# lubaroli/sigsvgd

Measured on AMD Instinct MI355X. Metric: SVGD iters/sec, sig-kernel N=1024 T=64 d=7, higher is better.
Workload: dtype f64 static kernel + f32 sweeps and contraction (mixed), f32 I/O

## Files before the change

### sigsvgd_amd/csrc/gram_fast.hip

```cpp
#include <cstdlib>

#include "gram_fast_kernel.h"

namespace sigsvgd {

bool fast_supported(int T, int d, int n) { return n == 0 && T >= 3 && T <= 64 && d <= 16; }

namespace {
inline int grad_nw(int T, int d) { return (d <= 8) ? 8 : 4; }
inline int grad_wg_per_cu(int T, int d) { return (d <= 8 && T <= 32) ? 3 : 1; }
GradGeom fast_geometry(int A, int B, int T, int d, bool sym, int off, int stride, bool fold)
{
    return grad_geometry(A, B, T * d, sym, off, stride, fold, grad_nw(T, d), (long long)device_cu_count() * grad_wg_per_cu(T, d));
}
}

int sym_tile_rows_fast(int T, int d) { return grad_nw(T, d); }

static bool fixed_windows(int T, int want_grad)
{
    if (T != 64 || !want_grad) return false;
    const char *e = getenv("SIGSVGD_SWEEP_WINDOWS");
    return !(e && e[0] == 't');
}

static bool wave_balance(int T, int d, int want_grad, bool sym)
{
    if (!sym || d > 8 || !fast_has_balance<8, true>() || !fixed_windows(T, want_grad)) return false;
    const char *e = getenv("SIGSVGD_WAVE_BALANCE");
    return !(e && e[0] == 'o' && e[1] == 'f');
}

WsPlan fast_plan(int A, int B, int T, int d, int want_grad, bool sym, int off, int stride, bool fold, int kind)
{
    WsPlan w;
    const bool rbf = kind == SIGSVGD_STATIC_RBF;
    w.fixed_windows = rbf && fixed_windows(T, want_grad) ? 1 : 0;
    w.wave_balance = rbf && wave_balance(T, d, want_grad, sym) ? 1 : 0;
    if (d <= 4) w.kflag = w.take(flag_area_bytes(A, B));
    if (want_grad) {
        w.g = fast_geometry(A, B, T, d, sym, off, stride, fold);
        w.rseg = w.take(w.g.rseg_bytes);
        w.cslab = w.take(w.g.cslab_bytes);
    }
    return w;
}

namespace {
int run(const GramProblem &p, const WsPlan &w, bool sym, const TileMap &own, void *out, int out64)
{
    unsigned char *base = nullptr;
    int rc = ws_base(p, w, "fast", base);
    if (rc) return rc;
    FastArgs a{};
    fill_sweep_args(a, p, w, base);
    a.tm = own;
    int tile_rows = 0;
    rc = p.kind == SIGSVGD_STATIC_RBF ? dispatch_variant<0>(p, a, w, out != nullptr, sym, tile_rows)
                                      : fast_radial_dispatch(p, a, w, out != nullptr, sym, tile_rows);
    if (rc) return rc;
    return finish_launch(p, w, base, sym, a.tm, tile_rows, out, out64);
}
}

int fast_launch(const GramProblem &p)
{
    const bool sym = (p.flags & SIGSVGD_FLAG_Y_IS_X) && p.A == p.B;
    const WsPlan w = fast_plan(p.A, p.B, p.T, p.d, p.gradX_out != nullptr, sym, 0, 1, false, p.kind);
    return run(p, w, sym, make_tilemap(1, 0, 1, false), p.gradX_out, p.dtype == SIGSVGD_F64);
}

int fast_sym_partial(const GramProblem &p, int tile_offset, int tile_stride, bool fold, double *grad_partial)
{
    const WsPlan w = fast_plan(p.A, p.B, p.T, p.d, 1, true, tile_offset, tile_stride, fold, p.kind);
    return run(p, w, true, make_tilemap((p.A + grad_nw(p.T, p.d) - 1) / grad_nw(p.T, p.d), tile_offset, tile_stride, fold),
               grad_partial, 1);
}

}

SIG_EXEC_DEBUG_GETTER(fast)
```

### sigsvgd_amd/csrc/gram_fast_kernel.h

```cpp
#pragma once

#include <type_traits>

#include "sig_common.h"

namespace sigsvgd {

#define SIG_PRIO(n)                                                          \
    if (!GRAD || !SYM || (RING == 32 && NW == 4)) __builtin_amdgcn_s_setprio(n);

template <int BAL>
__device__ __forceinline__ void bal_top(bool first)
{
    if constexpr (BAL != 0) {
        if (first) __builtin_amdgcn_s_setprio(1);
    }
}
template <int BAL, int AT>
__device__ __forceinline__ void bal_switch(bool first)
{
    if constexpr (BAL != 0 && (BAL & 3) == AT) {
        if (first) __builtin_amdgcn_s_setprio(0);
        else __builtin_amdgcn_s_setprio(1);
    }
// ... 271 lines not shown
template <int PFIX, int SIGMA0, int NS>
__device__ __forceinline__ void sweep_rev_fixed(float &cur, float &dnA, float &dnB, float &V, const float *g, float *ksl, const float r3)
{
    static_assert((NS == 8 || NS == 5) && SIGMA0 % 8 == 0 && SIGMA0 + NS <= 2 * PFIX - 1, "statement shape");
    float t, y;
    SIG_EXEC_MUST_BE_FULL("sweep_rev_fixed");
    if constexpr (NS == 8)
        asm volatile(SIG_REV_STEP_X("dnA", "dnB", "g7", "k7", SIG_WIN_FIX("7")) SIG_REV_STEP_X("dnB", "dnA", "g6", "k6", SIG_WIN_FIX("6"))
                     SIG_REV_STEP_X("dnA", "dnB", "g5", "k5", SIG_WIN_FIX("5")) SIG_REV_STEP_X("dnB", "dnA", "g4", "k4", SIG_WIN_FIX("4"))
                     SIG_REV_STEP_X("dnA", "dnB", "g3", "k3", SIG_WIN_FIX("3")) SIG_REV_STEP_X("dnB", "dnA", "g2", "k2", SIG_WIN_FIX("2"))
                     SIG_REV_STEP_X("dnA", "dnB", "g1", "k1", SIG_WIN_FIX("1")) SIG_REV_STEP_X("dnB", "dnA", "g0", "k0", SIG_WIN_FIX("0"))
                     "s_mov_b64 exec, -1\n\t"
                     : [cur] "+v"(cur), [dnA] "+v"(dnA), [dnB] "+v"(dnB), [V] "+v"(V), [t] "=&v"(t), [y] "=&v"(y),
                       [k0] "+v"(ksl[0]), [k1] "+v"(ksl[1]), [k2] "+v"(ksl[2]), [k3] "+v"(ksl[3]), [k4] "+v"(ksl[4]),
                       [k5] "+v"(ksl[5]), [k6] "+v"(ksl[6]), [k7] "+v"(ksl[7])
                     : [g0] "v"(g[0]), [g1] "v"(g[1]), [g2] "v"(g[2]), [g3] "v"(g[3]), [g4] "v"(g[4]), [g5] "v"(g[5]),
                       [g6] "v"(g[6]), [g7] "v"(g[7]), [r3] "s"(r3), SIG_WIN_OPS(0), SIG_WIN_OPS(1), SIG_WIN_OPS(2),
                       SIG_WIN_OPS(3), SIG_WIN_OPS(4), SIG_WIN_OPS(5), SIG_WIN_OPS(6), SIG_WIN_OPS(7));
    else
        asm volatile(SIG_REV_STEP_X("dnB", "dnA", "g4", "k4", SIG_WIN_FIX("4"))
                     SIG_REV_STEP_X("dnA", "dnB", "g3", "k3", SIG_WIN_FIX("3")) SIG_REV_STEP_X("dnB", "dnA", "g2", "k2", SIG_WIN_FIX("2"))
                     SIG_REV_STEP_X("dnA", "dnB", "g1", "k1", SIG_WIN_FIX("1")) SIG_REV_STEP_X("dnB", "dnA", "g0", "k0", SIG_WIN_FIX("0"))
                     "s_mov_b64 exec, -1\n\t"
                     : [cur] "+v"(cur), [dnA] "+v"(dnA), [dnB] "+v"(dnB), [V] "+v"(V), [t] "=&v"(t), [y] "=&v"(y),
                       [k0] "+v"(ksl[0]), [k1] "+v"(ksl[1]), [k2] "+v"(ksl[2]), [k3] "+v"(ksl[3]), [k4] "+v"(ksl[4])
                     : [g0] "v"(g[0]), [g1] "v"(g[1]), [g2] "v"(g[2]), [g3] "v"(g[3]), [g4] "v"(g[4]), [r3] "s"(r3),
                       SIG_WIN_OPS(0), SIG_WIN_OPS(1), SIG_WIN_OPS(2), SIG_WIN_OPS(3), SIG_WIN_OPS(4));
}
template <int PFIX, int S0, int S1>
__device__ __forceinline__ void sweep_fwd_fixed_round(float &cur, float &upA, float &upB, float &V, const float *Dsl, float *Ksl, const float r3)
{
    if constexpr (S0 < S1) {
        sweep_fwd_fixed<PFIX, S0, (S1 - S0 < 8 ? S1 - S0 : 8)>(cur, upA, upB, V, Dsl + (S0 & 63), Ksl + (S0 & 63), r3);
        sweep_fwd_fixed_round<PFIX, S0 + 8, S1>(cur, upA, upB, V, Dsl, Ksl, r3);
    }
}
template <int PFIX, int S0, int S1>
__device__ __forceinline__ void sweep_rev_fixed_round(float &cur, float &dnA, float &dnB, float &V, const float *Dsl, float *Ksl, const float r3)
{
    if constexpr (S0 < S1) {
        sweep_rev_fixed_round<PFIX, S0 + 8, S1>(cur, dnA, dnB, V, Dsl, Ksl, r3);
        sweep_rev_fixed<PFIX, S0, (S1 - S0 < 8 ? S1 - S0 : 8)>(cur, dnA, dnB, V, Dsl + (S0 & 63), Ksl + (S0 & 63), r3);
    }
}

template <int RING>
__device__ __forceinline__ double resweep_fwd_fp64(const float (&Dsl)[RING], int P, int lrow)
{
    double cur = 1.0, upprev = 1.0;
    asm volatile("" : "+v"(lrow), "+s"(P));
    const bool rowv = lrow < P;
#pragma unroll
    for (int s0 = 0; s0 < 2 * RING - 3; s0 += 8) {
        if (s0 <= 2 * P - 2) {
#pragma unroll
            for (int s = s0; s < s0 + 8 && s < 2 * RING - 3; ++s) {
                const double up = dpp_shr1_one(cur);
                float gf = Dsl[s & (RING - 1)];
                asm volatile("" : "+v"(gf));
                const double g = (double)gf;
                const double t = cur + up;
                const double nw = (t - upprev) + g * __builtin_fma(g, t + upprev, 1.7320508075688772 * t);
                cur = (rowv && (unsigned)(s - lrow) < (unsigned)P) ? nw : cur;
                upprev = up;
            }
        }
    }
    return cur;
}

__device__ __forceinline__ double rsqrt_ge1(double x)
{
    const double y = __builtin_amdgcn_rsq(x);
    const double e = __builtin_fma(-(x * y), y, 1.0);
    return __builtin_fma(y * e, __builtin_fma(e, 0.375, 0.5), y);
}

constexpr int GS_STRIDE = 65;
constexpr int GS_WAVE = 64 * GS_STRIDE;
using f32x2 = __attribute__((ext_vector_type(2))) float;

__device__ __forceinline__ int gs_index(int slot, int lane) { return slot * GS_STRIDE + lane; }

template <int DPAD, int NW, bool GRAD, bool SYM, bool LP, int RING = 64, int PFIX = 0, int BAL = 0, int RADIAL = 0>
__global__ __launch_bounds__(NW * 64) __attribute__((amdgpu_waves_per_eu(
    GRAD ? ((RING == 32 && NW == 4 && DPAD <= 8) ? 3 : 1) : ((DPAD <= 8) ? 3 : 2),
    GRAD ? ((RING == 32 && NW == 4 && DPAD <= 8) ? 3 : 2) : ((DPAD <= 8) ? 3 : 2)))) void gram_fast_kernel(FastArgsOf<RADIAL> a)
{
    constexpr int DC = LP ? DPAD - 1 : DPAD;
    constexpr int NT = NW * 64;
    constexpr int RM = RING - 1;
    constexpr int RPW = (RING == 32) ? 2 : 1;
    constexpr int NWR = NW * RPW;
    static_assert(RADIAL == 0 || (PFIX == 0 && BAL == 0), "the radial kinds: general windows, no wave balance");
    static_assert(BAL == 0 || (GRAD && SYM && RING == 64 && NW == 8 && PFIX != 0 && (BAL & 3) != 0 && BAL < 8),
                  "wave balance: the symmetric gradient kernels with fixed windows on 8-wave workgroups (the ones SIG_PRIO leaves alone)");
    constexpr int YDS = DPAD + 2;
    constexpr int YFS = (DPAD == 4) ? 12 : DPAD + 4;
    constexpr int GSW = RING * GS_STRIDE;
    __shared__ float Gs_all[GRAD ? NW * GSW : 1];
    __shared__ __align__(16) double yd[2 * RING * YDS];
    __shared__ double ynd[2 * RING];
    __shared__ double yref[DPAD];
    __shared__ __align__(16) float yf[GRAD ? 2 * RING * YFS : 1];

    const int tid = threadIdx.x, lane = tid & 63;
    const int wave = __builtin_amdgcn_readfirstlane(tid >> 6);
    const int lrow = lane & RM;
    const bool bal_first = (BAL & 4) ? wave < NW / 2 : wave >= NW / 2;
    const int T = a.T, d = a.d, P = T - 1, io64 = a.io64;
#ifdef SIGSVGD_PHASE_STAMPS
    unsigned long long ph_[SIG_FAST_PHASES] = {0, 0, 0, 0, 0, 0, 0, 0, 0}, tlast_ = __builtin_amdgcn_s_memtime();
#endif
    int j0 = 0, j1 = 0;
    float *Gs = Gs_all + (GRAD ? wave * GSW : 0);
    const double inv_h = a.inv_h;
    const float m2h = (float)(-2.0 * inv_h * 3.46410161513775459);

    float Ksl[RING];
    double gacc[DPAD];
    double xraw[DPAD];

    constexpr int EPT = (64 * DPAD + NT - 1) / NT;
    constexpr bool RAW_STAGE = GRAD && SYM && RING == 64 && DPAD == 8;
    struct RawElem { unsigned lo, hi; };
    RawElem raw_v[EPT], raw_r[EPT];
    double stage_v[EPT], stage_r[EPT];
    auto load_raw = [&](const void *b, size_t idx) -> RawElem {
        const char *p = static_cast<const char *>(b) + (idx << (io64 ? 3 : 2));
        RawElem r;
        r.lo = *reinterpret_cast<const unsigned *>(p);
        r.hi = 0u;
        if (io64) r.hi = *reinterpret_cast<const unsigned *>(p + 4);
        return r;
    };
    auto raw_value = [&](const RawElem &r) -> double {
        return io64 ? __hiloint2double((int)r.hi, (int)r.lo) : (double)__uint_as_float(r.lo);
    };
    auto stage_load = [&](int j) {
#pragma unroll
        for (int k = 0; k < EPT; ++k) {
            const int e = tid + k * NT;
            const int t = e / DPAD, c = e % DPAD;
            const bool ok = e < RING * DPAD && t < T && c < d && j < a.B;
            if constexpr (RAW_STAGE) {
                raw_v[k] = raw_r[k] = RawElem{0u, 0u};
                if (ok) {
                    raw_v[k] = load_raw(a.Y, ((size_t)j * T + t) * d + c);
                    raw_r[k] = load_raw(a.Y, (size_t)j * T * d + c);
                }
            } else {
                stage_v[k] = ok ? load_any(a.Y, ((size_t)j * T + t) * d + c, io64) : 0.0;
                stage_r[k] = ok ? load_any(a.Y, (size_t)j * T * d + c, io64) : 0.0;
            }
        }
    };
    const double nscale = RADIAL ? inv_h : -inv_h * 1.4426950408889634074;
    auto stage_store = [&]() {
#pragma unroll
        for (int k = 0; k < EPT; ++k) {
            const int e = tid + k * NT;
            if (e < RING * DPAD) {
                const int t = e / DPAD, c = e % DPAD;
                if constexpr (RAW_STAGE) {
                    stage_v[k] = raw_value(raw_v[k]);
                    stage_r[k] = raw_value(raw_r[k]);
                }
                const double v = stage_v[k] - stage_r[k];
                if (!(LP && c == DPAD - 1)) {
                    yd[t * YDS + c] = v;
                    yd[(t + RING) * YDS + c] = v;
                }
                if (GRAD) {
                    yf[t * YFS + c] = (float)v;
                    yf[(t + RING) * YFS + c] = (float)v;
                }
                if (t == 0) yref[c] = stage_r[k];
                double s = v * v * nscale;
#pragma unroll
                for (int off = 1; off < DPAD; off <<= 1) s += __shfl_xor(s, off, 64);
                if (c == 0) {
                    ynd[t] = s;
                    ynd[t + RING] = s;
                    if (LP) {
                        yd[t * YDS + DPAD - 1] = s;
                        yd[(t + RING) * YDS + DPAD - 1] = s;
                    }
                }
            }
        }
    };

    const long long it0 = a.nitems * blockIdx.x / gridDim.x, it1 = a.nitems * (blockIdx.x + 1) / gridDim.x;
    int remaining = (int)(it1 - it0);
    long long item = it0;
    int kq = 0, cstart = 0;
    {
        long long rem = it0;
        for (;; ++kq) {
            const int cn = a.B - (SYM ? a.tm.tile_of(kq) * NWR : 0);
            if (rem < cn) break;
            rem -= cn;
        }
        cstart = (int)rem;
    }
    bool staged = false;
    while (remaining > 0) {
    const int itile = a.tm.tile_of(kq);
    const int cfirst = SYM ? itile * NWR : 0;
    const int ncol = min(a.B - cfirst - cstart, remaining);
    const int jnext_tile = SYM ? a.tm.tile_of(kq + 1) * NWR : 0;
    const bool more_tiles = remaining > ncol;
    const int i0 = itile * NWR + wave * RPW;
    const int i = (RING == 32) ? i0 + (lane >> 5) : i0;
    const bool row_ok = i < a.A;
#pragma unroll
    for (int c = 0; c < DPAD; ++c) {
        gacc[c] = 0.0;
        xraw[c] = (row_ok && lrow < T && c < d) ? load_any(a.X, ((size_t)i * T + lrow) * d + c, io64) : 0.0;
    }
    if constexpr (RAW_STAGE) {
#pragma unroll
        for (int c = 0; c < DPAD; ++c) asm volatile("" : "+v"(xraw[c]));
    }
    j0 = cfirst + cstart;
    j1 = j0 + ncol;
    if (!staged) {
        staged = true;
        stage_load(j0);
        stage_store();
        __syncthreads();
    }

    for (int j = j0; j < j1; ++j) {
        const bool pair_ok = i0 < a.A && (!SYM || j >= i0);
        const bool mine = row_ok && (!SYM || j >= i);
        const bool last = j + 1 == j1;
        const bool more = !last || more_tiles;
        if (more) stage_load(last ? jnext_tile : j + 1);

        float Dsl[RING];

        SIG_STAMP(0)
        SIG_PRIO(3)
        if (pair_ok) {
            bal_top<BAL>(bal_first);
            double xs[DPAD];
            double xn = 0.0;
#pragma unroll
            for (int c = 0; c < DPAD; ++c) {
                const double xc = (lrow < T && c < d) ? xraw[c] - yref[c] : 0.0;
                xn = __builtin_fma(xc, xc, xn);
                xs[c] = xc * (-2.0 * nscale);
            }
            if constexpr (RADIAL) xn = xn * nscale;
            else
            xn = __builtin_fma(xn, nscale, -1.79248125036057809);

            {
                double g0 = 0.0, g1 = 0.0, gprev = 0.0, rdprev = 0.0;
                const double *ybase = yd + (RING - lrow) * YDS;
                const double *nbase = ynd + (RING - lrow);
                double ynx[DPAD], nnx;
#pragma unroll
                for (int c = 0; c < DPAD; ++c) ynx[c] = ybase[c];
                nnx = LP ? 0.0 : nbase[0];
#pragma unroll
                for (int t = 0; t < RING + 2; ++t) {
                    double g;
                    if (t < RING) {
                        double ycu[DPAD];
#pragma unroll
                        for (int c = 0; c < DPAD; ++c) ycu[c] = ynx[c];
                        double e2 = LP ? xn + ycu[DPAD - 1] : xn + nnx;
                        if (t < RING - 1) {
                            const double *yr = ybase + (t + 1) * YDS;
#pragma unroll
                            for (int c = 0; c < DPAD; ++c) ynx[c] = yr[c];
                            if (!LP) nnx = nbase[t + 1];
                        }
#pragma unroll
                        for (int c = 0; c < DC; ++c) e2 = __builtin_fma(xs[c], ycu[c], e2);
                        if constexpr (RADIAL) {
                            const double ki = rsqrt_ge1(1.0 + (e2 < 0.0 ? 0.0 : e2)), ki2 = ki * ki;
                            const bool rq = a.kind == SIGSVGD_STATIC_RQ;
                            g = (rq ? ki2 : ki) * 0.28867513459481288225;
                            if (GRAD) Gs[gs_index(t, lane)] = (float)((rq ? ki2 : 0.5 * ki) * (ki2 * 0.28867513459481288225));
                        } else {
                        g = exp2_p7(e2);
                        if (GRAD) Gs[gs_index(t, lane)] = (float)g;
                        }
                        if (t == 0) g0 = g;
                        if (t == 1) g1 = g;
                    } else {
                        g = (t == RING) ? g0 : g1;
                    }
                    const double rd = g - gprev;
                    gprev = g;
                    if (t >= 2) {
                        const double nb = dpp_shl1_zero(rd);
                        Dsl[(t - 2) & RM] = (float)(nb - rdprev);
                        asm volatile("" : "+v"(Dsl[(t - 2) & RM]));
                    }
                    rdprev = rd;
                    __builtin_amdgcn_sched_barrier(0);
                }
            }

            SIG_STAMP(1)
            SIG_PRIO(2)
            bal_switch<BAL, 1>(bal_first);
            float kf_keep = 0.f;
            bool x0_keep = false, x1_keep = false;
            {
                float cur = 1.f, upA = 1.f, upB = 1.f, V = 0.f, km = 1.f, sd = 0.f;
                const int smax = 2 * P - 2;
                if (GRAD) {
#pragma unroll
                    for (int k = 0; k < RING; ++k) Ksl[k] = 0.f;
                }
                if constexpr (PFIX != 0) {
                    static_assert(GRAD && RING == 64 && PFIX == 63, "fixed windows: gradient kernels of the 64-slot ring at T = 64");
                    float r3 = 1.7320508075688772f;
                    asm volatile("" : "+s"(r3));
                    sweep_fwd_fixed_round<PFIX, 0, 64>(cur, upA, upB, V, Dsl, Ksl, r3);
                    asm volatile("" : "+s"(r3));
                    sweep_fwd_fixed_round<PFIX, 64, 2 * PFIX - 1>(cur, upA, upB, V, Dsl, Ksl, r3);
                } else
                for (int rnd = 0; rnd < (RING == 64 ? 2 : 1); ++rnd) {
                    if (rnd * 64 > smax) break;
                    float r3 = 1.7320508075688772f;
                    asm volatile("" : "+s"(r3));
                    const unsigned long long *mk = (RING == 64 ? SWEEP_MASK.m[P] : SWEEP_MASK32.m[P]) + rnd * 64;
#pragma unroll
                    for (int k0 = 0; k0 < 64; k0 += 8)
                        sweep_fwd8<GRAD ? 0 : (DPAD == 4 ? 2 : 1)>(cur, upA, upB, V, &Dsl[k0 & RM], &Ksl[k0 & RM], mk + k0, r3, km, sd);
                }
                if (GRAD) {
                    km = fabsf(cur);
#pragma unroll
                    for (int k = 0; k < RING; k += 2) km = max3_abs(km, Ksl[k], Ksl[k + 1]);
                }
                float kf = __int_as_float(__builtin_amdgcn_readlane(__float_as_int(cur), P - 1));
                if (RING == 32) {
                    const float kf1 = __int_as_float(__builtin_amdgcn_readlane(__float_as_int(cur), 32 + P - 1));
                    kf = (lane >> 5) ? kf1 : kf;
                }
                bool x0 = false, x1 = false;
                if constexpr (DPAD == 4) {
                    if (a.kflag) {
                        const float kden = fmaxf(fabsf(kf), 0.1f);
                        bool fl = km > (d == 1 ? 2.f : 4.f) * kden;
                        if constexpr (!GRAD) {
                            const float wsum = wave_sum_dpp<RING == 64>(sd);
                            float sds = __int_as_float(__builtin_amdgcn_readlane(__float_as_int(wsum), 63));
                            if (RING == 32) {
                                const float s0 = __int_as_float(__builtin_amdgcn_readlane(__float_as_int(wsum), 31));
                                sds = (lane >> 5) ? sds : s0;
                            }
                            fl = fl || sds * 3.46410161513775459f * fmaxf(km, 1.f) > 300.f * kden;
                        }
                        const unsigned long long xbal = __builtin_amdgcn_ballot_w64(mine && kf == kf && fl);
                        x0 = (RING == 64) ? xbal != 0 : (unsigned)xbal != 0u;
                        x1 = (xbal >> 32) != 0;
                    }
                }
                if (lrow == P - 1 && mine) {
                    store_any(a.K, (size_t)i * a.B + j, (double)cur, io64);
                    if (SYM && j != i) store_any(a.K, (size_t)j * a.B + i, (double)cur, io64);
                    if constexpr (DPAD == 4 && !GRAD) {
                        if (a.kflag) a.kflag[(size_t)i * a.B + j] = (RING == 32 && (lane >> 5)) ? x1 : x0;
                    }
                }
                kf_keep = kf;
                x0_keep = x0;
                x1_keep = x1;
                if (__builtin_expect(__builtin_amdgcn_ballot_w64(mine && km > 4.f * fmaxf(fabsf(kf), 0.1f)) != 0, 0)) {
                    const double k64 = resweep_fwd_fp64<RING>(Dsl, P, lrow);
                    if (lrow == P - 1 && mine) {
                        store_any(a.K, (size_t)i * a.B + j, k64, io64);
                        if (SYM && j != i) store_any(a.K, (size_t)j * a.B + i, k64, io64);
                    }
                }
            }

            SIG_STAMP(2)
            SIG_PRIO(1)
            bal_switch<BAL, 2>(bal_first);
            if (GRAD) {
                float w_ij = 1.f, w_ji = 1.f;
                if (!mine) {
                    w_ij = 0.f; w_ji = 0.f;
                } else if (a.go) {
                    w_ij = (float)load_any(a.go, (size_t)i * a.B + j, io64);
                    if (SYM || a.symw) w_ji = (float)load_any(a.go, (size_t)j * a.B + i, io64);
                    if (a.symw) { w_ij += w_ji; w_ji = w_ij; }
                } else if (a.symw) {
                    w_ij = 2.f; w_ji = 2.f;
                }
                const float wcol = (mine && j != i) ? w_ji : 0.f;
                float cur = 1.f, downA = 1.f, downB = 1.f, V = 0.f;
                float Sb = 0.f, eprev = 0.f;
                f32x2 acc[DPAD / 2];
#pragma unroll
                for (int c = 0; c < DPAD / 2; ++c) acc[c] = f32x2{0.f, 0.f};
                const int smax = 2 * P - 2;

                f32x2 xc2[DPAD / 2];
#pragma unroll
                for (int c = 0; c < DPAD / 2; ++c) {
                    const bool ok0 = lrow < T && 2 * c < d, ok1 = lrow < T && 2 * c + 1 < d;
                    xc2[c] = f32x2{ok0 ? (float)(xraw[2 * c] - yref[2 * c]) : 0.f,
                                   ok1 ? (float)(xraw[2 * c + 1] - yref[2 * c + 1]) : 0.f};
                }
                float tacc[DPAD];
#pragma unroll
                for (int c = 0; c < DPAD; ++c) tacc[c] = 0.f;

                int yfrow = RING - lrow;
                int gsoff = (GRAD ? wave * GSW : 0) + lane;
                auto grad_part = [&](float Snew, bool accumulate, float gcu, const f32x2 *ycu) {
                    const float e = Sb - Snew;
                    const float up = shfl_up_zero(e);
                    const float R = eprev - up;
                    eprev = e;
                    Sb = Snew;
                    if (!accumulate) return;
                    const float rg = R * gcu;
                    const f32x2 rg2 = {rg, rg};
                    f32x2 df[DPAD / 2];
#pragma unroll
                    for (int c = 0; c < DPAD / 2; ++c) df[c] = xc2[c] - ycu[c];
#pragma unroll
                    for (int c = 0; c < DPAD / 2; ++c) acc[c] = __builtin_elementwise_fma(rg2, df[c], acc[c]);
#pragma unroll
                    for (int c = 0; c < DPAD / 2; ++c) asm volatile("" : "+v"(acc[c]));
                    if (SYM) {
                        const float rgc = (RING == 32) ? rg * wcol : rg;
                        const f32x2 rgc2 = {rgc, rgc};
#pragma unroll
                        for (int c = 0; c < DPAD / 2; ++c) {
                            const f32x2 pr = rgc2 * df[c];
                            tacc[2 * c] = add_rol1(tacc[2 * c], pr[0]);
                            if (2 * c + 1 < DC) tacc[2 * c + 1] = add_rol1(tacc[2 * c + 1], pr[1]);
                        }
#pragma unroll
                        for (int c = 0; c < DPAD; ++c) asm volatile("" : "+v"(tacc[c]));
                    }
                };

                if constexpr (PFIX != 0) {
                    asm volatile("" : "+v"(yfrow), "+v"(gsoff));
                    float r3 = 1.7320508075688772f;
                    asm volatile("" : "+s"(r3));
                    sweep_rev_fixed_round<PFIX, 64, 2 * PFIX - 1>(cur, downA, downB, V, Dsl, Ksl, r3);
                    bal_switch<BAL, 3>(bal_first);
                    asm volatile("" : "+v"(yfrow), "+v"(gsoff));
                    asm volatile("" : "+s"(r3));
                    sweep_rev_fixed_round<PFIX, 0, 64>(cur, downA, downB, V, Dsl, Ksl, r3);
                } else
                for (int rnd = (RING == 64 ? 1 : 0); rnd >= 0; --rnd) {
                    if (rnd * 64 > smax) continue;
                    asm volatile("" : "+v"(yfrow), "+v"(gsoff));
                    float r3 = 1.7320508075688772f;
                    asm volatile("" : "+s"(r3));
                    const unsigned long long *mk = (RING == 64 ? SWEEP_MASK.m[P] : SWEEP_MASK32.m[P]) + rnd * 64;
#pragma unroll
                    for (int k0 = 56; k0 >= 0; k0 -= 8) sweep_rev8(cur, downA, downB, V, &Dsl[k0 & RM], &Ksl[k0 & RM], mk + k0, r3);
                }

                if constexpr (DPAD == 4) {
                    if (a.kflag) {
                        float cs = 0.f;
#pragma unroll
                        for (int k = 0; k < RING; ++k) cs = __builtin_fmaf(fabsf(Ksl[k]), fabsf(Dsl[k]), cs);
                        const float wsum = wave_sum_dpp<RING == 64>(cs);
                        float c1 = __int_as_float(__builtin_amdgcn_readlane(__float_as_int(wsum), 63));
                        if (RING == 32) {
                            const float c10 = __int_as_float(__builtin_amdgcn_readlane(__float_as_int(wsum), 31));
                            c1 = (lane >> 5) ? c1 : c10;
                        }
                        const bool ill = kf_keep == kf_keep && c1 * 3.46410161513775459f > 150.f * fmaxf(fabsf(kf_keep), 0.1f);
                        if (lrow == P - 1 && mine)
                            a.kflag[(size_t)i * a.B + j] = (((RING == 32 && (lane >> 5)) ? x1_keep : x0_keep) || ill) ? 1 : 0;
                    }
                }
                SIG_STAMP(3)
                SIG_PRIO(0)
                float gnx = 0.f, Svn = Ksl[RM];
                f32x2 ynx[DPAD / 2];
#pragma unroll
                for (int c = 0; c < DPAD / 2; ++c) ynx[c] = f32x2{0.f, 0.f};
#pragma unroll
                for (int it = 0; it < RING + 2; ++it) {
                    const float Sv = Svn, gcu = gnx;
                    f32x2 ycu[DPAD / 2];
#pragma unroll
                    for (int c = 0; c < DPAD / 2; ++c) ycu[c] = ynx[c];
                    if (it + 1 < RING + 2) {
                        Svn = Ksl[(RING - 2 - it) & RM];
                        if (it + 1 >= 2) {
                            const int k2n = (RING - it) & RM;
                            gnx = Gs_all[gsoff + k2n * GS_STRIDE];
                            const f32x2 *yr = reinterpret_cast<const f32x2 *>(yf + (yfrow + k2n) * YFS);
#pragma unroll
                            for (int c = 0; c < DPAD / 2; ++c) ynx[c] = yr[c];
                        }
                    }
                    grad_part(Sv, it >= 2, gcu, ycu);
                    __builtin_amdgcn_sched_barrier(0);
                }

                SIG_STAMP(4)
#pragma unroll
                for (int c = 0; c < DPAD; ++c) {
                    gacc[c] += (double)(w_ij * m2h * acc[c / 2][c % 2]);
                }

                if (SYM) {
                    const int ncol = (RING - lrow) & RM;
                    const float wpark = (ncol <= P) ? ((RING == 32) ? -m2h : -(wcol * m2h)) : 0.f;
                    float *pk = Gs + ((RING == 32 ? (lane >> 5) * RING : 0) + ncol) * DPAD;
#pragma unroll
                    for (int c = 0; c < DPAD; ++c) pk[c] = wpark * tacc[c];
                }
            }
        } else if (GRAD && SYM) {
#pragma unroll
            for (int c = 0; c < DPAD; ++c) Gs[lane * DPAD + c] = 0.f;
        }
        if constexpr (RAW_STAGE) {
#pragma unroll
            for (int k = 0; k < EPT; ++k)
                asm volatile("" : "+v"(raw_v[k].lo), "+v"(raw_v[k].hi), "+v"(raw_r[k].lo), "+v"(raw_r[k].hi));
        }
        bal_end<BAL>(bal_first);
        SIG_STAMP(5)
#ifndef SIG_EXPERIMENT_NO_PAIR_BARRIER
        __syncthreads();
#endif
        SIG_STAMP(6)
        if (GRAD && SYM) {
            const float inv_d = 1.0f / (float)d;
            float *dst = a.cslab + (size_t)item * (T * d);
            for (int e = tid; e < T * d; e += NT) {
                const int n = (int)(((float)e + 0.5f) * inv_d), c = e - n * d;
                float s = 0.f;
#pragma unroll
                for (int w = 0; w < NW; ++w) {
                    s += Gs_all[w * GSW + n * DPAD + c];
                    if (RING == 32) s += Gs_all[w * GSW + (RING + n) * DPAD + c];
                }
                dst[e] = s;
            }
        }
        ++item;
        if (more) stage_store();
        SIG_STAMP(7)
#ifndef SIG_EXPERIMENT_NO_PAIR_BARRIER
        __syncthreads();
#endif
        SIG_STAMP(8)
    }

    if (GRAD && row_ok && lrow < T) {
        const int rslot = wave * RPW + (RING == 32 ? (lane >> 5) : 0);
        double *dst = a.rseg + (((size_t)(kq + (int)blockIdx.x)) * NWR + rslot) * (size_t)(T * d) + lrow * d;
#pragma unroll
        for (int c = 0; c < DPAD; ++c)
            if (c < d) dst[c] = gacc[c];
    }
    remaining -= ncol;
    ++kq;
    cstart = 0;
    }
#ifdef SIGSVGD_PHASE_STAMPS
    SIG_STAMP(0)
    if (lane == 0 && a.stamps)
        for (int k = 0; k < SIG_FAST_PHASES; ++k) atomicAdd(&a.stamps[(wave >= NW / 2 ? SIG_FAST_PHASES : 0) + k], ph_[k]);
#endif
}

#ifndef SIG_EXPERIMENT_BALANCE
#define SIG_EXPERIMENT_BALANCE 6
#endif
constexpr int FAST_BAL = SIG_EXPERIMENT_BALANCE;
template <int DPAD, bool SYM>
constexpr bool fast_has_balance() { return FAST_BAL != 0 && SYM && DPAD <= 8; }

int fast_radial_dispatch(const GramProblem &p, FastArgs &a, const WsPlan &w, bool grad, bool sym, int &tile_rows);

namespace {
template <int DPAD, int NW, bool SYM, bool LP, int RING, int RADIAL>
void launch_grad(bool fix, bool bal, dim3 grid, dim3 block, hipStream_t stream, const FastArgsOf<RADIAL> &a)
{
    if constexpr (RADIAL == 0 && RING == 64 && NW == (DPAD <= 8 ? 8 : 4)) {
        if constexpr (fast_has_balance<DPAD, SYM>()) {
            if (fix && bal) {
                hipLaunchKernelGGL((gram_fast_kernel<DPAD, NW, true, SYM, LP, RING, 63, FAST_BAL>), grid, block, 0, stream, a);
                return;
            }
        }
        if (fix) {
            hipLaunchKernelGGL((gram_fast_kernel<DPAD, NW, true, SYM, LP, RING, 63>), grid, block, 0, stream, a);
            return;
        }
    }
    hipLaunchKernelGGL((gram_fast_kernel<DPAD, NW, true, SYM, LP, RING, 0, 0, RADIAL>), grid, block, 0, stream, a);
}

template <int RADIAL, int DPAD, int NW, int RING = 64>
int launch_variant(const GramProblem &p, FastArgs &a, const WsPlan &w, bool grad, bool sym, int &tile_rows)
{
    constexpr int NWR = NW * (RING == 32 ? 2 : 1);
    tile_rows = NWR;
    const TileMap tm = make_tilemap((p.A + NWR - 1) / NWR, a.tm.off, a.tm.stride, a.tm.fold != 0);
    if (tm.owned <= 0) return SIGSVGD_OK;
    const long long total = tm.start(tm.owned, p.B, NWR, sym ? 1 : 0);
    if (total <= 0) return SIGSVGD_OK;
    const int ncu = device_cu_count();
    a.tm = tm;
    a.nitems = total;
#ifdef SIGSVGD_PHASE_STAMPS
    a.stamps = phase_stamps_begin(p.stream);
#endif
    const long long resident = (long long)ncu * (grad ? ((RING == 32 && NW == 4 && DPAD <= 8) ? 3 : 1) : (NW == 4 ? ((DPAD <= 8) ? 3 : 2) : 1));
    dim3 grid((unsigned)(total < resident ? total : resident), 1);
    dim3 block(NW * 64);
    if (grad) {
        const GradGeom &g = w.g;
        if (g.NW != NWR || g.grid != (int)grid.x || g.nitems != total) {
            set_error("fast: launch geometry mismatch (rows per tile %d/%d grid %d/%u items %lld/%lld)", g.NW, NWR, g.grid, grid.x,
                      g.nitems, total);
            return SIGSVGD_E_BADARG;
        }
    }
    constexpr bool HAS_LP = DPAD <= 8;
    const bool lp = HAS_LP && grad && p.d == DPAD - 1;
    FastArgsOf<RADIAL> ka{};
    static_cast<FastArgs &>(ka) = a;
    if constexpr (RADIAL != 0) ka.kind = p.kind;
    const bool fix = grad && w.fixed_windows && p.T == 64;
    const bool bal = fix && w.wave_balance;
    if (!grad && sym)
        hipLaunchKernelGGL((gram_fast_kernel<DPAD, NW, false, true, false, RING, 0, 0, RADIAL>), grid, block, 0, p.stream, ka);
    else if (!grad)
        hipLaunchKernelGGL((gram_fast_kernel<DPAD, NW, false, false, false, RING, 0, 0, RADIAL>), grid, block, 0, p.stream, ka);
    else if (sym && lp)
        launch_grad<DPAD, NW, true, HAS_LP, RING, RADIAL>(fix, bal, grid, block, p.stream, ka);
    else if (sym)
        launch_grad<DPAD, NW, true, false, RING, RADIAL>(fix, bal, grid, block, p.stream, ka);
    else if (lp)
        launch_grad<DPAD, NW, false, HAS_LP, RING, RADIAL>(fix, bal, grid, block, p.stream, ka);
    else
        launch_grad<DPAD, NW, false, false, RING, RADIAL>(fix, bal, grid, block, p.stream, ka);
    hipError_t e = hipGetLastError();
    if (e != hipSuccess) return hip_fail(e, "launch gram_fast_kernel");
#ifdef SIGSVGD_PHASE_STAMPS
    static const char *const nm[] = {"loop top", "phase 0+1 static kernel", "phase 2 forward sweep", "phase 3 reverse sweep",
                                      "phase 4 gradient pass", "pair epilogue", "barrier after the pair",
                                      "block sum + stage store", "second barrier"};
    static_assert(sizeof(nm) / sizeof(nm[0]) == SIG_FAST_PHASES, "one name per stamp slot");
    phase_stamps_report_halves(p.stream, a.stamps, nm, "[phase stamps] A=%d T=%d d=%d grad=%d sym=%d: ", p.A, p.T, p.d, (int)grad, (int)sym);
#endif
    return SIGSVGD_OK;
}

template <int RADIAL>
int dispatch_variant(const GramProblem &p, FastArgs &a, const WsPlan &w, bool grad, bool sym, int &tile_rows)
{
    if (!grad && p.d <= 4)
        return p.T <= 32 ? launch_variant<RADIAL, 4, 4, 32>(p, a, w, false, sym, tile_rows) : launch_variant<RADIAL, 4, 4>(p, a, w, false, sym, tile_rows);
    if (!grad && p.d <= 8)
        return p.T <= 32 ? launch_variant<RADIAL, 8, 4, 32>(p, a, w, false, sym, tile_rows) : launch_variant<RADIAL, 8, 4>(p, a, w, false, sym, tile_rows);
    if (p.d <= 4)
        return p.T <= 32 ? launch_variant<RADIAL, 4, 4, 32>(p, a, w, grad, sym, tile_rows) : launch_variant<RADIAL, 4, 8>(p, a, w, grad, sym, tile_rows);
    if (p.d <= 8)
        return p.T <= 32 ? launch_variant<RADIAL, 8, 4, 32>(p, a, w, grad, sym, tile_rows) : launch_variant<RADIAL, 8, 8>(p, a, w, grad, sym, tile_rows);
    return launch_variant<RADIAL, 16, 4>(p, a, w, grad, sym, tile_rows);
}
}
}
```

### sigsvgd_amd/csrc/sig_common.h

```cpp
#pragma once
#include <hip/hip_runtime.h>
#include <stdint.h>

#include <atomic>
#ifdef SIGSVGD_PHASE_STAMPS
#include <cstdarg>
#include <cstdio>
#endif

#include "../../include/sigsvgd_hip.h"

namespace sigsvgd {

constexpr int kWave = 64;

void set_error(const char *fmt, ...);
int hip_fail(hipError_t e, const char *what);

__device__ __forceinline__ double exp64(double a0)
{
    double a = fmin(fmax(a0, -1000.0), 700.0);
    const double kf = __builtin_rint(a * 1.4426950408889634074);
    double r = __builtin_fma(kf, -6.93147180369123816490e-01, a);
    r = __builtin_fma(kf, -1.90821492927058770002e-10, r);
// ... 191 lines not shown
    }
#else
#define SIG_EXEC_MUST_BE_FULL(what)
#define SIG_EXEC_DEBUG_GETTER(unit)
#endif

struct GramProblem {
    const void *X, *Y;
    int A, B, T, d, dtype;
    double inv_h;
    int n;
    int kind;
    unsigned flags;
    const void *grad_out;
    void *K_out;
    void *gradX_out;
    void *ws;
    size_t ws_bytes;
    hipStream_t stream;
};

struct LongProblem {
    const void *X, *Y;
    int A, B, TX, TY, d, dtype;
    double inv_h;
    int n;
    int kind;
    unsigned flags;
    const void *grad_out;
    void *K_out;
    void *gradX_out, *gradY_out;
    void *ws;
    size_t ws_bytes;
    hipStream_t stream;
};

struct TileMap {
    int off, stride, ntile, owned, m0, fold;
    __host__ __device__ int tile_of(int kq) const
    {
        return kq < m0 ? off + kq * stride : ntile - 1 - (off + (kq - m0) * stride);
    }
    __host__ __device__ int kq_of_tile(int ti) const
    {
        if (ti >= off && (ti - off) % stride == 0 && (ti - off) / stride < m0) return (ti - off) / stride;
        const int p = ntile - 1 - ti;
        if (p >= off && (p - off) % stride == 0 && (p - off) / stride < owned - m0) return m0 + (p - off) / stride;
        return -1;
    }
    __host__ __device__ long long start(int kq, int B, int NW, int sym) const
    {
        if (!sym) return (long long)kq * B;
        const long long k1 = kq < m0 ? kq : m0, k2 = kq - k1;
        long long s = k1 * B - (long long)NW * ((long long)stride * k1 * (k1 - 1) / 2 + (long long)off * k1);
        s += k2 * ((long long)B - (long long)(ntile - 1 - off) * NW) + (long long)NW * stride * k2 * (k2 - 1) / 2;
        return s;
    }
};
TileMap make_tilemap(int ntile, int off, int stride, bool fold);

struct GradGeom {
    int NW, grid;
    TileMap tm;
    long long nitems;
    size_t rseg_bytes, cslab_bytes;
};
int device_cu_count();
GradGeom grad_geometry(int A, int B, int TD, bool sym, int off, int stride, bool fold, int NW, long long resident);
int grad_reduce_launch(const GradGeom &g, const double *rseg, const float *cslab, void *out, int out64, int A, int B, int TD,
                       bool sym, hipStream_t stream);

struct WsArea {
    size_t off = 0, bytes = 0;
};
struct WsPlan {
    GradGeom g{};
    WsArea kflag;
    WsArea rseg, cslab;
    WsArea crec, rowg, dcache;
    WsArea wsk;
    WsArea counter, partials, colslab;
    int fixed_windows = 0;
    int wave_balance = 0;
    size_t end = 0;
    WsArea take(size_t bytes)
    {
        const WsArea a{end, bytes};
        end += bytes;
        return a;
    }
    size_t total() const { return end + 256; }
};
inline size_t flag_area_bytes(int A, int B) { return ((size_t)A * B + 255) & ~(size_t)255; }
template <typename T>
inline T *ws_at(unsigned char *base, const WsArea &a)
{
    return a.bytes ? reinterpret_cast<T *>(base + a.off) : nullptr;
}
int ws_base(const GramProblem &p, const WsPlan &w, const char *family, unsigned char *&base);
int finish_launch(const GramProblem &p, const WsPlan &w, unsigned char *base, bool sym, const TileMap &tm, int tile_rows,
                  void *out, int out64);

template <typename Args>
void fill_sweep_args(Args &a, const GramProblem &p, const WsPlan &w, unsigned char *base)
{
    a.X = p.X; a.Y = p.Y; a.go = p.grad_out; a.K = p.K_out;
    a.kflag = ws_at<unsigned char>(base, w.kflag); a.rseg = ws_at<double>(base, w.rseg); a.cslab = ws_at<float>(base, w.cslab);
    a.io64 = p.dtype == SIGSVGD_F64; a.A = p.A; a.B = p.B; a.T = p.T; a.d = p.d;
    a.symw = (p.flags & SIGSVGD_FLAG_SYM) ? 1 : 0; a.inv_h = p.inv_h;
}

template <auto KERNEL>
hipError_t raise_lds_limit()
{
    static std::atomic<unsigned long long> raised{0};
    int dev = 0;
    (void)hipGetDevice(&dev);
    if (dev < 0 || dev >= 64 || !((raised.load(std::memory_order_acquire) >> dev) & 1ull)) {
        hipError_t e = hipFuncSetAttribute(reinterpret_cast<const void *>(KERNEL), hipFuncAttributeMaxDynamicSharedMemorySize,
                                           160 * 1024);
        if (e != hipSuccess) return e;
        if (dev >= 0 && dev < 64) raised.fetch_or(1ull << dev, std::memory_order_release);
    }
    return hipSuccess;
}


int generic_plan(int A, int B, int T, int d, int n, int want_grad, bool sym, bool precise, bool any_size, WsPlan &w);
int generic_launch(const GramProblem &p, bool precise, bool any_size);
int generic_repair_launch(const GramProblem &p, const unsigned char *flags, bool sym, const TileMap &tm, int tile_rows);

bool fast_supported(int T, int d, int n);
WsPlan fast_plan(int A, int B, int T, int d, int want_grad, bool sym, int off = 0, int stride = 1, bool fold = false,
                 int kind = SIGSVGD_STATIC_RBF);
int fast_launch(const GramProblem &p);
int fast_sym_partial(const GramProblem &p, int tile_offset, int tile_stride, bool fold, double *grad_partial);
int sym_tile_rows_fast(int T, int d);

bool quad_supported(int T, int d, int n);
WsPlan quad_plan(int A, int B, int T, int d, int want_grad, bool sym, int off = 0, int stride = 1, bool fold = false);
int quad_launch(const GramProblem &p);
int quad_sym_partial(const GramProblem &p, int tile_offset, int tile_stride, bool fold, double *grad_partial);

bool dyad_supported(int T, int d, int n);
WsPlan dyad_plan(int A, int B, int T, int d, int want_grad, bool sym);
int dyad_launch(const GramProblem &p);

bool band_supported(int T, int d, int n);
int band_wg_per_cu(int T, int d, int n, bool serial);
WsPlan band_plan(int A, int B, int T, int d, int n, int want_grad, bool sym, bool serial);
int band_launch(const GramProblem &p, bool serial);

}
```

Baseline: 220.9.

## Offset younger half of waves by a pair with double-buffered staging

```diff
diff --git a/sigsvgd_amd/csrc/gram_fast.hip b/sigsvgd_amd/csrc/gram_fast.hip
--- a/sigsvgd_amd/csrc/gram_fast.hip
+++ b/sigsvgd_amd/csrc/gram_fast.hip
@@ -31,12 +31,20 @@
     return !(e && e[0] == 'o' && e[1] == 'f');
 }
 
+static bool half_offset(int T, int d, int want_grad, bool sym)
+{
+    if (!sym || d != 7 || !fast_has_half<8, true, true>() || !fixed_windows(T, want_grad)) return false;
+    const char *e = getenv("SIGSVGD_HALF_OFFSET");
+    return !(e && e[0] == 'o' && e[1] == 'f');
+}
+
 WsPlan fast_plan(int A, int B, int T, int d, int want_grad, bool sym, int off, int stride, bool fold, int kind)
 {
     WsPlan w;
     const bool rbf = kind == SIGSVGD_STATIC_RBF;
     w.fixed_windows = rbf && fixed_windows(T, want_grad) ? 1 : 0;
     w.wave_balance = rbf && wave_balance(T, d, want_grad, sym) ? 1 : 0;
+    w.half_offset = rbf && half_offset(T, d, want_grad, sym) ? 1 : 0;
     if (d <= 4) w.kflag = w.take(flag_area_bytes(A, B));
     if (want_grad) {
         w.g = fast_geometry(A, B, T, d, sym, off, stride, fold);
diff --git a/sigsvgd_amd/csrc/gram_fast_kernel.h b/sigsvgd_amd/csrc/gram_fast_kernel.h
--- a/sigsvgd_amd/csrc/gram_fast_kernel.h
+++ b/sigsvgd_amd/csrc/gram_fast_kernel.h
@@ -377,7 +377,7 @@
 
 __device__ __forceinline__ int gs_index(int slot, int lane) { return slot * GS_STRIDE + lane; }
 
-template <int DPAD, int NW, bool GRAD, bool SYM, bool LP, int RING = 64, int PFIX = 0, int BAL = 0, int RADIAL = 0>
+template <int DPAD, int NW, bool GRAD, bool SYM, bool LP, int RING = 64, int PFIX = 0, int BAL = 0, int RADIAL = 0, int HALF = 0>
 __global__ __launch_bounds__(NW * 64) __attribute__((amdgpu_waves_per_eu(
     GRAD ? ((RING == 32 && NW == 4 && DPAD <= 8) ? 3 : 1) : ((DPAD <= 8) ? 3 : 2),
     GRAD ? ((RING == 32 && NW == 4 && DPAD <= 8) ? 3 : 2) : ((DPAD <= 8) ? 3 : 2)))) void gram_fast_kernel(FastArgsOf<RADIAL> a)
@@ -390,19 +390,27 @@
     static_assert(RADIAL == 0 || (PFIX == 0 && BAL == 0), "the radial kinds: general windows, no wave balance");
     static_assert(BAL == 0 || (GRAD && SYM && RING == 64 && NW == 8 && PFIX != 0 && (BAL & 3) != 0 && BAL < 8),
                   "wave balance: the symmetric gradient kernels with fixed windows on 8-wave workgroups (the ones SIG_PRIO leaves alone)");
+    static_assert(HALF == 0 || (GRAD && SYM && LP && DPAD == 8 && RING == 64 && NW == 8 && PFIX != 0 && BAL == 0 && RADIAL == 0),
+                  "half offset: the symmetric 7-of-8-channel gradient kernel with fixed windows on 8-wave workgroups; a schedule of its own");
     constexpr int YDS = DPAD + 2;
     constexpr int YFS = (DPAD == 4) ? 12 : DPAD + 4;
-    constexpr int GSW = RING * GS_STRIDE;
+    constexpr int GSS = HALF ? 64 : GS_STRIDE;
+    constexpr int GSW = RING * GSS;
     __shared__ float Gs_all[GRAD ? NW * GSW : 1];
     __shared__ __align__(16) double yd[2 * RING * YDS];
-    __shared__ double ynd[2 * RING];
-    __shared__ double yref[DPAD];
-    __shared__ __align__(16) float yf[GRAD ? 2 * RING * YFS : 1];
+    __shared__ double ynd[HALF ? 1 : 2 * RING];
+    constexpr int YFB = 2 * RING * YFS;
+    __shared__ double yref[HALF ? 2 * DPAD : DPAD];
+    __shared__ __align__(16) float yf[GRAD ? (HALF ? 2 : 1) * YFB : 1];
+    __shared__ float ypark[HALF ? (NW / 2) * RING * DC : 1];
+    __shared__ float ycarry[HALF ? RING * DC : 1];
 
     const int tid = threadIdx.x, lane = tid & 63;
     const int wave = __builtin_amdgcn_readfirstlane(tid >> 6);
     const int lrow = lane & RM;
     const bool bal_first = (BAL & 4) ? wave < NW / 2 : wave >= NW / 2;
+    const bool half_younger = HALF != 0 && wave >= NW / 2;
+    int pb = 0;
     const int T = a.T, d = a.d, P = T - 1, io64 = a.io64;
 #ifdef SIGSVGD_PHASE_STAMPS
     unsigned long long ph_[SIG_FAST_PHASES] = {0, 0, 0, 0, 0, 0, 0, 0, 0}, tlast_ = __builtin_amdgcn_s_memtime();
@@ -451,7 +459,7 @@
         }
     };
     const double nscale = RADIAL ? inv_h : -inv_h * 1.4426950408889634074;
-    auto stage_store = [&]() {
+    auto stage_store = [&](int buf) {
 #pragma unroll
         for (int k = 0; k < EPT; ++k) {
             const int e = tid + k * NT;
@@ -467,16 +475,19 @@
                     yd[(t + RING) * YDS + c] = v;
                 }
                 if (GRAD) {
-                    yf[t * YFS + c] = (float)v;
-                    yf[(t + RING) * YFS + c] = (float)v;
-                }
-                if (t == 0) yref[c] = stage_r[k];
+                    float *yfb = yf + (HALF ? buf * YFB : 0);
+                    yfb[t * YFS + c] = (float)v;
+                    yfb[(t + RING) * YFS + c] = (float)v;
+                }
+                if (t == 0) yref[(HALF ? buf * DPAD : 0) + c] = stage_r[k];
                 double s = v * v * nscale;
 #pragma unroll
                 for (int off = 1; off < DPAD; off <<= 1) s += __shfl_xor(s, off, 64);
                 if (c == 0) {
-                    ynd[t] = s;
-                    ynd[t + RING] = s;
+                    if constexpr (!HALF) {
+                        ynd[t] = s;
+                        ynd[t + RING] = s;
+                    }
                     if (LP) {
                         yd[t * YDS + DPAD - 1] = s;
                         yd[(t + RING) * YDS + DPAD - 1] = s;
@@ -523,7 +534,7 @@
     if (!staged) {
         staged = true;
         stage_load(j0);
-        stage_store();
+        stage_store(pb);
         __syncthreads();
     }
 
@@ -535,6 +546,60 @@
         if (more) stage_load(last ? jnext_tile : j + 1);
 
         float Dsl[RING];
+        const double *yrefp = yref + (HALF ? pb * DPAD : 0);
+        auto pair_sync = [&]() __attribute__((always_inline)) {
+            SIG_STAMP(5)
+#ifndef SIG_EXPERIMENT_NO_PAIR_BARRIER
+            __syncthreads();
+#endif
+            SIG_STAMP(6)
+            if constexpr (HALF != 0) {
+                const float inv_d = 1.0f / (float)d;
+                const bool pend = j > j0;
+                float *dstp = a.cslab + (size_t)(item - 1) * (T * d);
+                for (int e = tid; e < T * d; e += NT) {
+                    const int n = (int)(((float)e + 0.5f) * inv_d), c = e - n * d;
+                    if (pend) {
+                        float s = ycarry[e];
+#pragma unroll
+                        for (int w = 0; w < NW / 2; ++w) s += ypark[w * RING * DC + e];
+                        dstp[e] = s;
+                    }
+                    float s = 0.f;
+#pragma unroll
+                    for (int w = 0; w < NW / 2; ++w) s += Gs_all[w * GSW + n * DPAD + c];
+                    ycarry[e] = s;
+                }
+            } else if (GRAD && SYM) {
+                const float inv_d = 1.0f / (float)d;
+                float *dst = a.cslab + (size_t)item * (T * d);
+                for (int e = tid; e < T * d; e += NT) {
+                    const int n = (int)(((float)e + 0.5f) * inv_d), c = e - n * d;
+                    float s = 0.f;
+#pragma unroll
+                    for (int w = 0; w < NW; ++w) {
+                        s += Gs_all[w * GSW + n * DPAD + c];
+                        if (RING == 32) s += Gs_all[w * GSW + (RING + n) * DPAD + c];
+                    }
+                    dst[e] = s;
+                }
+            }
+            ++item;
+            if (more) stage_store(HALF ? pb ^ 1 : 0);
+            SIG_STAMP(7)
+#ifndef SIG_EXPERIMENT_NO_PAIR_BARRIER
+            __syncthreads();
+#endif
+            SIG_STAMP(8)
+        };
+        auto younger_sync = [&]() __attribute__((always_inline)) {
+            if constexpr (RAW_STAGE) {
+#pragma unroll
+                for (int k = 0; k < EPT; ++k)
+                    asm volatile("" : "+v"(raw_v[k].lo), "+v"(raw_v[k].hi), "+v"(raw_r[k].lo), "+v"(raw_r[k].hi));
+            }
+            pair_sync();
+        };
 
         SIG_STAMP(0)
         SIG_PRIO(3)
@@ -544,7 +609,7 @@
             double xn = 0.0;
 #pragma unroll
             for (int c = 0; c < DPAD; ++c) {
-                const double xc = (lrow < T && c < d) ? xraw[c] - yref[c] : 0.0;
+                const double xc = (lrow < T && c < d) ? xraw[c] - yrefp[c] : 0.0;
                 xn = __builtin_fma(xc, xc, xn);
                 xs[c] = xc * (-2.0 * nscale);
             }
@@ -580,10 +645,10 @@
                             const double ki = rsqrt_ge1(1.0 + (e2 < 0.0 ? 0.0 : e2)), ki2 = ki * ki;
                             const bool rq = a.kind == SIGSVGD_STATIC_RQ;
                             g = (rq ? ki2 : ki) * 0.28867513459481288225;
-                            if (GRAD) Gs[gs_index(t, lane)] = (float)((rq ? ki2 : 0.5 * ki) * (ki2 * 0.28867513459481288225));
+                            if (GRAD) Gs[t * GSS + lane] = (float)((rq ? ki2 : 0.5 * ki) * (ki2 * 0.28867513459481288225));
                         } else {
                         g = exp2_p7(e2);
-                        if (GRAD) Gs[gs_index(t, lane)] = (float)g;
+                        if (GRAD) Gs[t * GSS + lane] = (float)g;
                         }
                         if (t == 0) g0 = g;
                         if (t == 1) g1 = g;
@@ -682,6 +747,10 @@
             SIG_STAMP(2)
             SIG_PRIO(1)
             bal_switch<BAL, 2>(bal_first);
+            if constexpr (HALF != 0) {
+                if (half_younger) younger_sync();
+                __builtin_amdgcn_s_setprio(1);
+            }
             if (GRAD) {
                 float w_ij = 1.f, w_ji = 1.f;
                 if (!mine) {
@@ -705,14 +774,14 @@
 #pragma unroll
                 for (int c = 0; c < DPAD / 2; ++c) {
                     const bool ok0 = lrow < T && 2 * c < d, ok1 = lrow < T && 2 * c + 1 < d;
-                    xc2[c] = f32x2{ok0 ? (float)(xraw[2 * c] - yref[2 * c]) : 0.f,
-                                   ok1 ? (float)(xraw[2 * c + 1] - yref[2 * c + 1]) : 0.f};
+                    xc2[c] = f32x2{ok0 ? (float)(xraw[2 * c] - yrefp[2 * c]) : 0.f,
+                                   ok1 ? (float)(xraw[2 * c + 1] - yrefp[2 * c + 1]) : 0.f};
                 }
                 float tacc[DPAD];
 #pragma unroll
                 for (int c = 0; c < DPAD; ++c) tacc[c] = 0.f;
 
-                int yfrow = RING - lrow;
+                int yfrow = RING - lrow + (HALF ? pb * 2 * RING : 0);
                 int gsoff = (GRAD ? wave * GSW : 0) + lane;
                 auto grad_part = [&](float Snew, bool accumulate, float gcu, const f32x2 *ycu) {
                     const float e = Sb - Snew;
@@ -796,7 +865,7 @@
                         Svn = Ksl[(RING - 2 - it) & RM];
                         if (it + 1 >= 2) {
                             const int k2n = (RING - it) & RM;
-                            gnx = Gs_all[gsoff + k2n * GS_STRIDE];
+                            gnx = Gs_all[gsoff + k2n * GSS];
                             const f32x2 *yr = reinterpret_cast<const f32x2 *>(yf + (yfrow + k2n) * YFS);
 #pragma unroll
                             for (int c = 0; c < DPAD / 2; ++c) ynx[c] = yr[c];
@@ -815,14 +884,26 @@
                 if (SYM) {
                     const int ncol = (RING - lrow) & RM;
                     const float wpark = (ncol <= P) ? ((RING == 32) ? -m2h : -(wcol * m2h)) : 0.f;
+                    if (HALF != 0 && half_younger) {
+                        float *pk = ypark + ((wave - NW / 2) * RING + ncol) * DC;
+#pragma unroll
+                        for (int c = 0; c < DC; ++c) pk[c] = wpark * tacc[c];
+                    } else {
                     float *pk = Gs + ((RING == 32 ? (lane >> 5) * RING : 0) + ncol) * DPAD;
 #pragma unroll
                     for (int c = 0; c < DPAD; ++c) pk[c] = wpark * tacc[c];
+                    }
                 }
             }
         } else if (GRAD && SYM) {
+            if (HALF != 0 && half_younger) {
+                younger_sync();
+#pragma unroll
+                for (int c = 0; c < DC; ++c) ypark[((wave - NW / 2) * RING + lane) * DC + c] = 0.f;
+            } else {
 #pragma unroll
             for (int c = 0; c < DPAD; ++c) Gs[lane * DPAD + c] = 0.f;
+            }
         }
         if constexpr (RAW_STAGE) {
 #pragma unroll
@@ -830,32 +911,19 @@
                 asm volatile("" : "+v"(raw_v[k].lo), "+v"(raw_v[k].hi), "+v"(raw_r[k].lo), "+v"(raw_r[k].hi));
         }
         bal_end<BAL>(bal_first);
-        SIG_STAMP(5)
-#ifndef SIG_EXPERIMENT_NO_PAIR_BARRIER
+        if constexpr (HALF != 0) __builtin_amdgcn_s_setprio(0);
+        if (!half_younger) pair_sync();
+        if constexpr (HALF != 0) pb ^= 1;
+    }
+    if constexpr (HALF != 0) {
         __syncthreads();
-#endif
-        SIG_STAMP(6)
-        if (GRAD && SYM) {
-            const float inv_d = 1.0f / (float)d;
-            float *dst = a.cslab + (size_t)item * (T * d);
-            for (int e = tid; e < T * d; e += NT) {
-                const int n = (int)(((float)e + 0.5f) * inv_d), c = e - n * d;
-                float s = 0.f;
-#pragma unroll
-                for (int w = 0; w < NW; ++w) {
-                    s += Gs_all[w * GSW + n * DPAD + c];
-                    if (RING == 32) s += Gs_all[w * GSW + (RING + n) * DPAD + c];
-                }
-                dst[e] = s;
-            }
-        }
-        ++item;
-        if (more) stage_store();
-        SIG_STAMP(7)
-#ifndef SIG_EXPERIMENT_NO_PAIR_BARRIER
-        __syncthreads();
-#endif
-        SIG_STAMP(8)
+        float *dstp = a.cslab + (size_t)(item - 1) * (T * d);
+        for (int e = tid; e < T * d; e += NT) {
+            float s = ycarry[e];
+#pragma unroll
+            for (int w = 0; w < NW / 2; ++w) s += ypark[w * RING * DC + e];
+            dstp[e] = s;
+        }
     }
 
     if (GRAD && row_ok && lrow < T) {
@@ -883,13 +951,22 @@
 template <int DPAD, bool SYM>
 constexpr bool fast_has_balance() { return FAST_BAL != 0 && SYM && DPAD <= 8; }
 
+template <int DPAD, bool SYM, bool LP>
+constexpr bool fast_has_half() { return SYM && LP && DPAD == 8; }
+
 int fast_radial_dispatch(const GramProblem &p, FastArgs &a, const WsPlan &w, bool grad, bool sym, int &tile_rows);
 
 namespace {
 template <int DPAD, int NW, bool SYM, bool LP, int RING, int RADIAL>
-void launch_grad(bool fix, bool bal, dim3 grid, dim3 block, hipStream_t stream, const FastArgsOf<RADIAL> &a)
+void launch_grad(bool fix, bool bal, bool half, dim3 grid, dim3 block, hipStream_t stream, const FastArgsOf<RADIAL> &a)
 {
     if constexpr (RADIAL == 0 && RING == 64 && NW == (DPAD <= 8 ? 8 : 4)) {
+        if constexpr (fast_has_half<DPAD, SYM, LP>()) {
+            if (fix && half) {
+                hipLaunchKernelGGL((gram_fast_kernel<DPAD, NW, true, SYM, LP, RING, 63, 0, 0, 1>), grid, block, 0, stream, a);
+                return;
+            }
+        }
         if constexpr (fast_has_balance<DPAD, SYM>()) {
             if (fix && bal) {
                 hipLaunchKernelGGL((gram_fast_kernel<DPAD, NW, true, SYM, LP, RING, 63, FAST_BAL>), grid, block, 0, stream, a);
@@ -937,18 +1014,19 @@
     if constexpr (RADIAL != 0) ka.kind = p.kind;
     const bool fix = grad && w.fixed_windows && p.T == 64;
     const bool bal = fix && w.wave_balance;
+    const bool half = fix && w.half_offset;
     if (!grad && sym)
         hipLaunchKernelGGL((gram_fast_kernel<DPAD, NW, false, true, false, RING, 0, 0, RADIAL>), grid, block, 0, p.stream, ka);
     else if (!grad)
         hipLaunchKernelGGL((gram_fast_kernel<DPAD, NW, false, false, false, RING, 0, 0, RADIAL>), grid, block, 0, p.stream, ka);
     else if (sym && lp)
-        launch_grad<DPAD, NW, true, HAS_LP, RING, RADIAL>(fix, bal, grid, block, p.stream, ka);
+        launch_grad<DPAD, NW, true, HAS_LP, RING, RADIAL>(fix, bal, half, grid, block, p.stream, ka);
     else if (sym)
-        launch_grad<DPAD, NW, true, false, RING, RADIAL>(fix, bal, grid, block, p.stream, ka);
+        launch_grad<DPAD, NW, true, false, RING, RADIAL>(fix, bal, half, grid, block, p.stream, ka);
     else if (lp)
-        launch_grad<DPAD, NW, false, HAS_LP, RING, RADIAL>(fix, bal, grid, block, p.stream, ka);
+        launch_grad<DPAD, NW, false, HAS_LP, RING, RADIAL>(fix, bal, half, grid, block, p.stream, ka);
     else
-        launch_grad<DPAD, NW, false, false, RING, RADIAL>(fix, bal, grid, block, p.stream, ka);
+        launch_grad<DPAD, NW, false, false, RING, RADIAL>(fix, bal, half, grid, block, p.stream, ka);
     hipError_t e = hipGetLastError();
     if (e != hipSuccess) return hip_fail(e, "launch gram_fast_kernel");
 #ifdef SIGSVGD_PHASE_STAMPS
diff --git a/sigsvgd_amd/csrc/sig_common.h b/sigsvgd_amd/csrc/sig_common.h
--- a/sigsvgd_amd/csrc/sig_common.h
+++ b/sigsvgd_amd/csrc/sig_common.h
@@ -297,6 +297,7 @@
     WsArea counter, partials, colslab;
     int fixed_windows = 0;
     int wave_balance = 0;
+    int half_offset = 0;
     size_t end = 0;
     WsArea take(size_t bytes)
     {
```

After: 231.2 (median of 6 runs). 1.05x the previous value.
